# eridgd/WCT-TF

Hardware: AMD Instinct MI355X
Metric: stylized frames/sec @512x512, 5-level relu5->1 pipeline, alpha=0.8 (higher is better)
Workload: dtype f16

## Files before the change

### wct_tf_amd/csrc/conv_wino.hip

```cpp
#include "common.h"

namespace {
typedef unsigned int u32x4 __attribute__((ext_vector_type(4)));
typedef _Float16 h2 __attribute__((ext_vector_type(2)));
constexpr int TW = 16;
constexpr int PITCH = 20;
constexpr int BK = 32;

__device__ __forceinline__ half8 pk_sub(half8 a, half8 b) {
  u32x4 ua = __builtin_bit_cast(u32x4, a), ub = __builtin_bit_cast(u32x4, b), r;
#pragma unroll
  for (int i = 0; i < 4; ++i) {
    unsigned o;
    asm("v_pk_add_f16 %0, %1, %2 neg_lo:[0,1] neg_hi:[0,1]" : "=v"(o) : "v"(ua[i]), "v"(ub[i]));
    r[i] = o;
  }
  return __builtin_bit_cast(half8, r);
}

__device__ __forceinline__ int reflect_idx(int i, int n) {
  if (i < 0) i = -i;
  if (i >= n) i = 2 * n - 2 - i;
  i = i < 0 ? 0 : i;
  return i >= n ? n - 1 : i;
}

template <int TH, int BN, int WM, int WN, bool IL>
__global__ __launch_bounds__(256, TH >= 16 ? 1 : 2)
void conv3x3_wino_kernel(ConvArgs p, int tiles_x, int n_tiles) {
  constexpr int PR = TH / 2;
  constexpr int MT = (PR / 2) / WM;
  constexpr int NT = (BN / 32) / WN;
  constexpr int G = 256 / PR;
  constexpr int SL = (72 + G - 1) / G;
  constexpr int PATCH_BYTES = PR * 4 * PITCH * 64;
  constexpr int DUMP_OFF = 2 * PATCH_BYTES;
  constexpr int PF_TAP = 5;
  static_assert(PR % 2 == 0 && (PR / 2) % WM == 0 && 256 % PR == 0 && WM * WN == 4, "tile shape");

  extern __shared__ __attribute__((aligned(16))) unsigned char smem[];
  const int tid = threadIdx.x, lane = tid & 63, wave = tid >> 6;
  const int wm = wave / WN, wn = wave % WN;
  int bid = blockIdx.x;
  const int ntile = bid % n_tiles;
  bid /= n_tiles;
  const int tx = bid % tiles_x, ty = bid / tiles_x;
  const int b = blockIdx.y;
  const int y0 = ty * TH, x0 = tx * TW, n0 = ntile * BN;

  const int Hin = p.upsample ? p.H / 2 : p.H;
  const int Win = p.upsample ? p.W / 2 : p.W;
  const half_t* xb = p.x + (size_t)b * Hin * Win * p.Cin;
  const __amdgpu_buffer_rsrc_t w_rsrc = __builtin_amdgcn_make_buffer_rsrc((void*)p.w_wino, 0, 0x7FFFFFFF, 0x00020000);
  const __amdgpu_buffer_rsrc_t x_rsrc = __builtin_amdgcn_make_buffer_rsrc((void*)xb, 0, 0x7FFFFFFF, 0x00020000);

  const int lpr = tid / G, ls = tid % G;
  unsigned row_off[4], col_off[SL], dst_off[SL];
  bool slot_ok[SL];
#pragma unroll
  for (int i = 0; i < 4; ++i) {
    int iy = reflect_idx(y0 + 2 * lpr - 1 + i, p.H);
    if (p.upsample) iy >>= 1;
    row_off[i] = (unsigned)(iy * Win) * p.Cin * 2;
  }
#pragma unroll
  for (int j = 0; j < SL; ++j) {
    const int slot = ls + j * G;
    slot_ok[j] = slot < 72;
    const int px = slot_ok[j] ? slot >> 2 : 0, piece = slot & 3;
    int ix = reflect_idx(x0 - 1 + px, p.W);
    if (p.upsample) ix >>= 1;
    col_off[j] = (unsigned)(ix * p.Cin + piece * 8) * 2;
    dst_off[j] = ((lpr * 4 * PITCH + px) * 4 + (piece ^ ((px >> 2) & 3))) * 16;
    if (IL && !slot_ok[j]) dst_off[j] = DUMP_OFF + tid * 16;
  }
  u32x4 raw[SL][4];
  auto load_rows = [&](int chunk) {
#pragma unroll
    for (int j = 0; j < SL; ++j)
#pragma unroll
      for (int i = 0; i < 4; ++i)
        raw[j][i] = __builtin_amdgcn_raw_buffer_load_b128(x_rsrc, row_off[i] + col_off[j], chunk * BK * 2, 0);
  };
  auto park_rows = [&](int buf) {
#pragma unroll
    for (int j = 0; j < SL; ++j) {
      const half8 d0 = __builtin_bit_cast(half8, raw[j][0]), d1 = __builtin_bit_cast(half8, raw[j][1]);
      const half8 d2 = __builtin_bit_cast(half8, raw[j][2]), d3 = __builtin_bit_cast(half8, raw[j][3]);
      const half8 t0 = pk_sub(d0, d2), t1 = d1 + d2, t2 = pk_sub(d2, d1), t3 = pk_sub(d1, d3);
      if (slot_ok[j]) {
        unsigned char* d = smem + buf * PATCH_BYTES + dst_off[j];
        *reinterpret_cast<half8*>(d) = t0;
        *reinterpret_cast<half8*>(d + PITCH * 64) = t1;
        *reinterpret_cast<half8*>(d + 2 * PITCH * 64) = t2;
        *reinterpret_cast<half8*>(d + 3 * PITCH * 64) = t3;
      }
    }
  };

  const int frag_px = lane & 15, frag_pr = (lane & 31) >> 4, kgrp = lane >> 5;
  int rd_base[3][2];
#pragma unroll
  for (int kx = 0; kx < 3; ++kx)
#pragma unroll
    for (int ks = 0; ks < 2; ++ks) {
      const int px = frag_px + kx;
      rd_base[kx][ks] = (((wm * MT * 2 + frag_pr) * 4) * PITCH + px) * 64 + (((ks * 2 + kgrp) ^ ((px >> 2) & 3)) * 16);
    }
  const int c16 = p.Cin >> 4;
  unsigned wfrag[NT];
#pragma unroll
  for (int nt = 0; nt < NT; ++nt) wfrag[nt] = (((n0 >> 5) + wn * NT + nt) * 12 * c16 * 512 + lane * 8) * 2;

  f32x16 acc[4][NT][MT];
#pragma unroll
  for (int nt = 0; nt < NT; ++nt) {
    f32x4 bv[4];
#pragma unroll
    for (int rq = 0; rq < 4; ++rq) bv[rq] = *reinterpret_cast<const f32x4*>(p.bias + n0 + (wn * NT + nt) * 32 + 8 * rq + 4 * kgrp);
#pragma unroll
    for (int f = 0; f < 4; ++f)
#pragma unroll
      for (int mt = 0; mt < MT; ++mt)
#pragma unroll
        for (int r = 0; r < 16; ++r) acc[f][nt][mt][r] = f == 1 ? bv[r >> 2][r & 3] : 0.f;
  }

  const int n_chunks = p.Cin / BK;
  half8 wf[3][NT][2];
  half8 bf[IL ? 3 : 2][2][MT];
  auto load_w = [&](half8 (&dst)[NT][2], int tap12, int chunk) {
    const int soff = (tap12 * c16 + chunk * 2) * 1024;
#pragma unroll
    for (int nt = 0; nt < NT; ++nt)
#pragma unroll
      for (int ks = 0; ks < 2; ++ks)
        dst[nt][ks] = __builtin_bit_cast(half8, __builtin_amdgcn_raw_buffer_load_b128(w_rsrc, wfrag[nt] + ks * 1024, soff, 0));
  };
  auto read_b = [&](half8 (&dst)[2][MT], int f, int kx, int buf) {
#pragma unroll
    for (int ks = 0; ks < 2; ++ks)
#pragma unroll
      for (int mt = 0; mt < MT; ++mt)
        dst[ks][mt] = *reinterpret_cast<const half8*>(smem + buf * PATCH_BYTES + rd_base[kx][ks] + (mt * 8 + f) * PITCH * 64);
  };

  if constexpr (IL) {
    constexpr int NM = 2 * MT * NT;
    constexpr int NR = 2 * NT + 2 * MT;
#ifndef WINO_LT0
#define WINO_LT0 1
#define WINO_PT0 6
#endif
    constexpr int LT0 = WINO_LT0, PT0 = WINO_PT0;
    static_assert(LT0 + SL <= PT0 && PT0 + SL <= 10, "staging schedule");
#ifndef WINO_WRING
#define WINO_WRING 4
#endif
#ifndef WINO_ABL
#define WINO_ABL 0
#endif
#ifndef WINO_RAW_AUX
#define WINO_RAW_AUX 0
#endif
    constexpr int ABL = WINO_ABL;
    constexpr int WR = WINO_WRING, WA = WR - 1;
    static_assert(24 % WR == 0, "ring");
    half8 wq[WR][NT][2];
    half8 tq[4];
    load_rows(0);
#pragma unroll
    for (int i = 0; i < WA; ++i) load_w(wq[i], i, 0);
#pragma unroll
    for (int j = 0; j < SL; ++j) {
      const half8 d0 = __builtin_bit_cast(half8, raw[j][0]), d1 = __builtin_bit_cast(half8, raw[j][1]);
      const half8 d2 = __builtin_bit_cast(half8, raw[j][2]), d3 = __builtin_bit_cast(half8, raw[j][3]);
      unsigned char* d = smem + dst_off[j];
      *reinterpret_cast<half8*>(d) = pk_sub(d0, d2);
      *reinterpret_cast<half8*>(d + PITCH * 64) = d1 + d2;
      *reinterpret_cast<half8*>(d + 2 * PITCH * 64) = pk_sub(d2, d1);
      *reinterpret_cast<half8*>(d + 3 * PITCH * 64) = pk_sub(d1, d3);
    }
    asm volatile("s_waitcnt lgkmcnt(0)\n\ts_barrier" ::: "memory");
    read_b(bf[0], 0, 0, 0);
    read_b(bf[1], 0, 1, 0);
#pragma unroll 1
    for (int pair = 0; pair < n_chunks; pair += 2) {
#pragma unroll
      for (int t = 0; t < 24; ++t) {
        const int tt = t % 12, chunk_i = pair + t / 12, buf = t / 12;
        const int f = tt / 3, kx = tt % 3;
        const int chunk_n = chunk_i + 1 < n_chunks ? chunk_i + 1 : chunk_i;
        const int t3 = (tt + WA) % 12, c3 = tt + WA >= 12 ? chunk_n : chunk_i;
        const int t1 = (tt + 2) % 12, buf1 = tt >= 10 ? buf ^ 1 : buf;
        const int soff3 = (t3 * c16 + c3 * 2) * 1024;
#pragma unroll
        for (int j = 0; j < NM; ++j) {
          const int ks = j / (MT * NT), mt = (j / NT) % MT, nt = j % NT;
          if (!(ABL & 4)) acc[f][nt][mt] = __builtin_amdgcn_mfma_f32_32x32x16_f16(wq[t % WR][nt][ks], bf[t % 3][ks][mt], acc[f][nt][mt], 0, 0, 0);
          else asm volatile("" :: "v"(wq[t % WR][nt][ks]), "v"(bf[t % 3][ks][mt]));
#pragma unroll
          for (int k = j * NR / NM; k < (j + 1) * NR / NM; ++k) {
            if (k < 2 * NT) {
              if (!(ABL & 1)) wq[(t + WA) % WR][k / 2][k % 2] =
                  __builtin_bit_cast(half8, __builtin_amdgcn_raw_buffer_load_b128(w_rsrc, wfrag[k / 2] + (k % 2) * 1024, soff3, 0));
            } else {
              const int kk = k - 2 * NT, ks1 = kk / MT, mt1 = kk % MT;
              if (!(ABL & 8)) bf[(t + 2) % 3][ks1][mt1] = *reinterpret_cast<const half8*>(smem + buf1 * PATCH_BYTES + rd_base[t1 % 3][ks1] + (mt1 * 8 + t1 / 3) * PITCH * 64);
            }
          }
          if (tt >= LT0 && tt < LT0 + SL) {
            const int sl = tt - LT0;
            if (j < 4 && !(ABL & 2)) raw[sl][j] = __builtin_amdgcn_raw_buffer_load_b128(x_rsrc, (ABL & 64) ? (lane & 3) * 16 + j * 64 + sl * 256 : row_off[j] + col_off[sl], (ABL & 32) ? 0 : chunk_n * BK * 2, WINO_RAW_AUX);
          }
          if (tt >= PT0 && tt < PT0 + SL && !(ABL & 16)) {
            const int sl = tt - PT0;
            {
#pragma unroll
              for (int it = j * 8 / NM; it < (j + 1) * 8 / NM; ++it) {
                const int fq = it >> 1;
                if ((it & 1) == 0) {
                  const half8 da = __builtin_bit_cast(half8, raw[sl][fq == 0 ? 0 : fq == 1 ? 1 : fq == 2 ? 2 : 1]);
                  const half8 db = __builtin_bit_cast(half8, raw[sl][fq == 0 ? 2 : fq == 1 ? 2 : fq == 2 ? 1 : 3]);
                  tq[fq] = fq == 1 ? da + db : pk_sub(da, db);
                } else {
                  *reinterpret_cast<half8*>(smem + (buf ^ 1) * PATCH_BYTES * (slot_ok[sl] ? 1 : 0) + dst_off[sl] + fq * PITCH * 64) = tq[fq];
                }
              }
            }
          }
          __builtin_amdgcn_sched_barrier(0);
        }
        if (tt == 9) asm volatile("s_waitcnt lgkmcnt(0)\n\ts_barrier" ::: "memory");
      }
    }
  } else {
  load_rows(0);
  load_w(wf[0], 0, 0);
  load_w(wf[1], 1, 0);
  park_rows(0);
  asm volatile("s_waitcnt lgkmcnt(0)\n\ts_barrier" ::: "memory");
  read_b(bf[0], 0, 0, 0);

#pragma unroll 1
  for (int pair = 0; pair < n_chunks; pair += 2) {
#pragma unroll
    for (int t = 0; t < 24; ++t) {
      const int tt = t % 12, chunk_i = pair + t / 12, buf = t / 12;
      const int f = tt / 3, kx = tt % 3;
      const bool more = chunk_i + 1 < n_chunks;
      {
        const int t2 = (tt + 2) % 12;
        const int c2 = tt + 2 >= 12 ? (more ? chunk_i + 1 : chunk_i) : chunk_i;
        load_w(wf[(t + 2) % 3], t2, c2);
      }
      if (tt == PF_TAP && more) load_rows(chunk_i + 1);
      if (tt != 11) read_b(bf[(t + 1) & 1], (tt + 1) / 3, (tt + 1) % 3, buf);
      else if (more) read_b(bf[(t + 1) & 1], 0, 0, buf ^ 1);
      __builtin_amdgcn_sched_barrier(0);
#pragma unroll
      for (int ks = 0; ks < 2; ++ks)
#pragma unroll
        for (int mt = 0; mt < MT; ++mt)
#pragma unroll
          for (int nt = 0; nt < NT; ++nt)
            acc[f][nt][mt] = __builtin_amdgcn_mfma_f32_32x32x16_f16(wf[t % 3][nt][ks], bf[t & 1][ks][mt], acc[f][nt][mt], 0, 0, 0);
      __builtin_amdgcn_sched_barrier(0);
      if (tt == 10 && more) {
        park_rows(buf ^ 1);
        asm volatile("s_waitcnt lgkmcnt(0)\n\ts_barrier" ::: "memory");
      }
    }
  }

  }
  constexpr int OOB = (int)0x80000000u;
  const int Ho = p.pool ? (p.H + 1) / 2 : p.H, Wo = p.pool ? (p.W + 1) / 2 : p.W;
  const unsigned img_elems = (unsigned)Ho * Wo * p.Cout;
  const __amdgpu_buffer_rsrc_t r16 = __builtin_amdgcn_make_buffer_rsrc((void*)(p.y16 + (size_t)b * img_elems), 0, img_elems * 2, 0x00020000);
  const float lo1 = p.relu ? 0.f : -__builtin_inff();
  const h2 lo2 = {(half_t)lo1, (half_t)lo1};
  const h2 zero2 = {(half_t)0.f, (half_t)0.f};
  const int ox = x0 + frag_px;
  const int chan = n0 + wn * NT * 32;
#pragma unroll
  for (int mt = 0; mt < MT; ++mt) {
    const int oy = y0 + ((wm * MT + mt) * 2 + frag_pr) * 2;
    const bool in0 = (oy < p.H) & (ox < p.W), in1 = (oy + 1 < p.H) & (ox < p.W);
    int off[2];
    if (p.pool) {
      off[0] = in0 && (frag_px & 1) == 0 ? (((oy >> 1) * Wo + (ox >> 1)) * p.Cout + chan + 8 * kgrp) * 2 : OOB;
      off[1] = OOB;
    } else {
      off[0] = in0 ? ((oy * p.W + ox) * p.Cout + chan + 8 * kgrp) * 2 : OOB;
      off[1] = in1 ? (((oy + 1) * p.W + ox) * p.Cout + chan + 8 * kgrp) * 2 : OOB;
    }
#pragma unroll
    for (int nt = 0; nt < NT; ++nt) {
      unsigned pk[2][4][2];
#pragma unroll
      for (int rq = 0; rq < 4; ++rq) {
        f32x4 e, o;
#pragma unroll
        for (int j = 0; j < 4; ++j) {
          const int r = rq * 4 + j;
          const float m0 = acc[0][nt][mt][r], m1 = acc[1][nt][mt][r], m2 = acc[2][nt][mt][r], m3 = acc[3][nt][mt][r];
          e[j] = (m0 + m1) + m2;
          o[j] = (m1 - m2) - m3;
        }
        h2 e0 = {(half_t)e[0], (half_t)e[1]}, e1 = {(half_t)e[2], (half_t)e[3]};
        h2 o0 = {(half_t)o[0], (half_t)o[1]}, o1 = {(half_t)o[2], (half_t)o[3]};
        e0 = __builtin_elementwise_max(e0, lo2); e1 = __builtin_elementwise_max(e1, lo2);
        o0 = __builtin_elementwise_max(o0, lo2); o1 = __builtin_elementwise_max(o1, lo2);
        if (p.pool) {
          h2 q[2] = {__builtin_elementwise_max(in0 ? e0 : zero2, in1 ? o0 : zero2), __builtin_elementwise_max(in0 ? e1 : zero2, in1 ? o1 : zero2)};
#pragma unroll
          for (int d = 0; d < 2; ++d) {
            const unsigned tq = __builtin_bit_cast(unsigned, q[d]);
            const h2 nb = __builtin_bit_cast(h2, __builtin_amdgcn_update_dpp(0, (int)tq, 0xB1, 0xF, 0xF, true));
            q[d] = __builtin_elementwise_max(q[d], nb);
          }
          e0 = q[0]; e1 = q[1];
        }
        pk[0][rq][0] = __builtin_bit_cast(unsigned, e0); pk[0][rq][1] = __builtin_bit_cast(unsigned, e1);
        pk[1][rq][0] = __builtin_bit_cast(unsigned, o0); pk[1][rq][1] = __builtin_bit_cast(unsigned, o1);
      }
#pragma unroll
      for (int par = 0; par < 2; ++par) {
#pragma unroll
        for (int m = 0; m < 2; ++m) {
          auto sx = __builtin_amdgcn_permlane32_swap(pk[par][2 * m][0], pk[par][2 * m + 1][0], false, false);
          auto sy = __builtin_amdgcn_permlane32_swap(pk[par][2 * m][1], pk[par][2 * m + 1][1], false, false);
          u32x4 ov = {sx[0], sy[0], sx[1], sy[1]};
          __builtin_amdgcn_raw_buffer_store_b128(ov, r16, off[par] + (nt * 32 + 16 * m) * 2, 0, 0);
        }
      }
    }
  }
}

template <int TH, int BN, int WM, int WN, bool IL = false>
int launch_wino_cfg(const ConvArgs& a, hipStream_t s) {
  const int tiles_x = cdiv(a.W, TW), tiles_y = cdiv(a.H, TH), n_tiles = a.Cout / BN;
  const size_t lds = 2 * (size_t)(TH / 2) * 4 * PITCH * 64 + (IL ? 8192 : 0);
  HIP_TRY(hipFuncSetAttribute(reinterpret_cast<const void*>(&conv3x3_wino_kernel<TH, BN, WM, WN, IL>),
                              hipFuncAttributeMaxDynamicSharedMemorySize, (int)lds));
  hipLaunchKernelGGL((conv3x3_wino_kernel<TH, BN, WM, WN, IL>), dim3(tiles_x * tiles_y * n_tiles, a.B), dim3(256), lds, s, a, tiles_x, n_tiles);
  HIP_TRY(hipGetLastError());
  return WCT_OK;
}
}

bool conv3x3_wino_takes(const ConvArgs& a) {
  return a.w_wino != nullptr && a.y16 != nullptr && a.y32 == nullptr && a.usum == nullptr && a.img1 == nullptr &&
         a.Cin % 64 == 0 && a.Cout % 64 == 0 && (!a.pool || a.relu);
}

int launch_conv3x3_wino(const ConvArgs& a, hipStream_t s) {
  ARG_CHECK(conv3x3_wino_takes(a) && a.H > 1 && a.W > 1 && a.B > 0);
  ARG_CHECK(!a.upsample || (a.H % 2 == 0 && a.W % 2 == 0));
  ARG_CHECK((size_t)a.H * a.W * a.Cin * 2 < ((size_t)1 << 31));
  ARG_CHECK((size_t)a.H * a.W * a.Cout * 2 < ((size_t)1 << 31));
  const long px16 = (long)cdiv(a.W, TW) * cdiv(a.H, 16) * a.B;
  const long px8 = (long)cdiv(a.W, TW) * cdiv(a.H, 8) * a.B;
  if (a.Cout % 128 == 0 && px16 * (a.Cout / 128) >= 256) return launch_wino_cfg<16, 128, 1, 4, true>(a, s);
  if (a.Cout % 128 == 0 && px8 * (a.Cout / 128) >= 256) return launch_wino_cfg<8, 128, 1, 4>(a, s);
  return launch_wino_cfg<8, 64, 2, 2>(a, s);
}
```

Before: 673.3.

## Specialize Winograd conv for nearest-upsampled input to drop duplicate rows

Adds an UP template variant of the F(2,3) Winograd conv kernel for convolutions whose input is 2x nearest-upsampled. Because row pairs are duplicated, the row input transform collapses to two loaded rows and three frequency planes instead of four, which cuts global loads, LDS footprint and the MFMA tap count by a quarter. Weight taps are remapped so the third plane uses the original fourth transformed weight. It is enabled by default and can be turned off with an environment variable, at the cost of a more complex staging schedule and constant tuning for the new path.

```diff
diff --git a/wct_tf_amd/csrc/conv_wino.hip b/wct_tf_amd/csrc/conv_wino.hip
--- a/wct_tf_amd/csrc/conv_wino.hip
+++ b/wct_tf_amd/csrc/conv_wino.hip
@@ -25,17 +25,23 @@
   return i >= n ? n - 1 : i;
 }
 
-template <int TH, int BN, int WM, int WN, bool IL>
+template <int TH, int BN, int WM, int WN, bool IL, bool UP>
 __global__ __launch_bounds__(256, TH >= 16 ? 1 : 2)
 void conv3x3_wino_kernel(ConvArgs p, int tiles_x, int n_tiles) {
+  constexpr int NF = UP ? 3 : 4;
+  constexpr int NTAP = NF * 3;
+  constexpr int NROW = UP ? 2 : 4;
+  constexpr int RPP = UP ? 2 : 4;
+  auto WF = [](int fi) constexpr { return UP && fi == 2 ? 3 : fi; };
   constexpr int PR = TH / 2;
   constexpr int MT = (PR / 2) / WM;
   constexpr int NT = (BN / 32) / WN;
   constexpr int G = 256 / PR;
-  constexpr int SL = (72 + G - 1) / G;
-  constexpr int PATCH_BYTES = PR * 4 * PITCH * 64;
+  constexpr int LR = UP ? PR + 1 : PR;
+  constexpr int SL = UP ? (LR * 72 + 255) / 256 : (72 + G - 1) / G;
+  constexpr int PATCH_BYTES = LR * RPP * PITCH * 64;
   constexpr int DUMP_OFF = 2 * PATCH_BYTES;
-  constexpr int PF_TAP = 5;
+  constexpr int PF_TAP = NTAP - 7;
   static_assert(PR % 2 == 0 && (PR / 2) % WM == 0 && 256 % PR == 0 && WM * WN == 4, "tile shape");
 
   extern __shared__ __attribute__((aligned(16))) unsigned char smem[];
@@ -48,52 +54,84 @@
   const int b = blockIdx.y;
   const int y0 = ty * TH, x0 = tx * TW, n0 = ntile * BN;
 
-  const int Hin = p.upsample ? p.H / 2 : p.H;
-  const int Win = p.upsample ? p.W / 2 : p.W;
+  const bool ups = UP || p.upsample;
+  const int Hin = ups ? p.H / 2 : p.H;
+  const int Win = ups ? p.W / 2 : p.W;
   const half_t* xb = p.x + (size_t)b * Hin * Win * p.Cin;
   const __amdgpu_buffer_rsrc_t w_rsrc = __builtin_amdgcn_make_buffer_rsrc((void*)p.w_wino, 0, 0x7FFFFFFF, 0x00020000);
   const __amdgpu_buffer_rsrc_t x_rsrc = __builtin_amdgcn_make_buffer_rsrc((void*)xb, 0, 0x7FFFFFFF, 0x00020000);
 
   const int lpr = tid / G, ls = tid % G;
-  unsigned row_off[4], col_off[SL], dst_off[SL];
+  unsigned row_off[4], col_off[SL], dst_off[SL], src_up[SL][2];
   bool slot_ok[SL];
-#pragma unroll
-  for (int i = 0; i < 4; ++i) {
-    int iy = reflect_idx(y0 + 2 * lpr - 1 + i, p.H);
-    if (p.upsample) iy >>= 1;
-    row_off[i] = (unsigned)(iy * Win) * p.Cin * 2;
-  }
-#pragma unroll
-  for (int j = 0; j < SL; ++j) {
-    const int slot = ls + j * G;
-    slot_ok[j] = slot < 72;
-    const int px = slot_ok[j] ? slot >> 2 : 0, piece = slot & 3;
-    int ix = reflect_idx(x0 - 1 + px, p.W);
-    if (p.upsample) ix >>= 1;
-    col_off[j] = (unsigned)(ix * p.Cin + piece * 8) * 2;
-    dst_off[j] = ((lpr * 4 * PITCH + px) * 4 + (piece ^ ((px >> 2) & 3))) * 16;
-    if (IL && !slot_ok[j]) dst_off[j] = DUMP_OFF + tid * 16;
-  }
+  if constexpr (!UP) {
+#pragma unroll
+    for (int i = 0; i < 4; ++i) {
+      int iy = reflect_idx(y0 + 2 * lpr - 1 + i, p.H);
+      if (ups) iy >>= 1;
+      row_off[i] = (unsigned)(iy * Win) * p.Cin * 2;
+    }
+#pragma unroll
+    for (int j = 0; j < SL; ++j) {
+      const int slot = ls + j * G;
+      slot_ok[j] = slot < 72;
+      const int px = slot_ok[j] ? slot >> 2 : 0, piece = slot & 3;
+      int ix = reflect_idx(x0 - 1 + px, p.W);
+      if (ups) ix >>= 1;
+      col_off[j] = (unsigned)(ix * p.Cin + piece * 8) * 2;
+      dst_off[j] = ((lpr * 4 * PITCH + px) * 4 + (piece ^ ((px >> 2) & 3))) * 16;
+      if (IL && !slot_ok[j]) dst_off[j] = DUMP_OFF + tid * 16;
+    }
+  } else {
+#pragma unroll
+    for (int j = 0; j < SL; ++j) {
+      const int item = tid + j * 256;
+      slot_ok[j] = item < LR * 72;
+      const int it = slot_ok[j] ? item : 0;
+      const int lr = it / 72, slot = it - lr * 72;
+      const int px = slot >> 2, piece = slot & 3;
+      const int ix = reflect_idx(x0 - 1 + px, p.W) >> 1;
+#pragma unroll
+      for (int i = 0; i < 2; ++i) {
+        const int iy = reflect_idx(y0 + 2 * lr - 1 + i, p.H) >> 1;
+        src_up[j][i] = (unsigned)((iy * Win + ix) * p.Cin + piece * 8) * 2;
+      }
+      dst_off[j] = ((lr * RPP * PITCH + px) * 4 + (piece ^ ((px >> 2) & 3))) * 16;
+      if (IL && !slot_ok[j]) dst_off[j] = DUMP_OFF + tid * 16;
+    }
+  }
+  auto src_off = [&](int j, int i) -> unsigned {
+    if constexpr (UP) return src_up[j][i]; else return row_off[i] + col_off[j];
+  };
   u32x4 raw[SL][4];
   auto load_rows = [&](int chunk) {
 #pragma unroll
     for (int j = 0; j < SL; ++j)
 #pragma unroll
-      for (int i = 0; i < 4; ++i)
-        raw[j][i] = __builtin_amdgcn_raw_buffer_load_b128(x_rsrc, row_off[i] + col_off[j], chunk * BK * 2, 0);
+      for (int i = 0; i < NROW; ++i)
+        raw[j][i] = __builtin_amdgcn_raw_buffer_load_b128(x_rsrc, src_off(j, i), chunk * BK * 2, 0);
   };
   auto park_rows = [&](int buf) {
 #pragma unroll
     for (int j = 0; j < SL; ++j) {
       const half8 d0 = __builtin_bit_cast(half8, raw[j][0]), d1 = __builtin_bit_cast(half8, raw[j][1]);
-      const half8 d2 = __builtin_bit_cast(half8, raw[j][2]), d3 = __builtin_bit_cast(half8, raw[j][3]);
-      const half8 t0 = pk_sub(d0, d2), t1 = d1 + d2, t2 = pk_sub(d2, d1), t3 = pk_sub(d1, d3);
-      if (slot_ok[j]) {
-        unsigned char* d = smem + buf * PATCH_BYTES + dst_off[j];
-        *reinterpret_cast<half8*>(d) = t0;
-        *reinterpret_cast<half8*>(d + PITCH * 64) = t1;
-        *reinterpret_cast<half8*>(d + 2 * PITCH * 64) = t2;
-        *reinterpret_cast<half8*>(d + 3 * PITCH * 64) = t3;
+      if constexpr (UP) {
+        const half8 t0 = pk_sub(d0, d1), t1 = d1 + d1;
+        if (slot_ok[j]) {
+          unsigned char* d = smem + buf * PATCH_BYTES + dst_off[j];
+          *reinterpret_cast<half8*>(d) = t0;
+          *reinterpret_cast<half8*>(d + PITCH * 64) = t1;
+        }
+      } else {
+        const half8 d2 = __builtin_bit_cast(half8, raw[j][2]), d3 = __builtin_bit_cast(half8, raw[j][3]);
+        const half8 t0 = pk_sub(d0, d2), t1 = d1 + d2, t2 = pk_sub(d2, d1), t3 = pk_sub(d1, d3);
+        if (slot_ok[j]) {
+          unsigned char* d = smem + buf * PATCH_BYTES + dst_off[j];
+          *reinterpret_cast<half8*>(d) = t0;
+          *reinterpret_cast<half8*>(d + PITCH * 64) = t1;
+          *reinterpret_cast<half8*>(d + 2 * PITCH * 64) = t2;
+          *reinterpret_cast<half8*>(d + 3 * PITCH * 64) = t3;
+        }
       }
     }
   };
@@ -105,21 +143,21 @@
 #pragma unroll
     for (int ks = 0; ks < 2; ++ks) {
       const int px = frag_px + kx;
-      rd_base[kx][ks] = (((wm * MT * 2 + frag_pr) * 4) * PITCH + px) * 64 + (((ks * 2 + kgrp) ^ ((px >> 2) & 3)) * 16);
+      rd_base[kx][ks] = (((wm * MT * 2 + frag_pr) * RPP) * PITCH + px) * 64 + (((ks * 2 + kgrp) ^ ((px >> 2) & 3)) * 16);
     }
   const int c16 = p.Cin >> 4;
   unsigned wfrag[NT];
 #pragma unroll
   for (int nt = 0; nt < NT; ++nt) wfrag[nt] = (((n0 >> 5) + wn * NT + nt) * 12 * c16 * 512 + lane * 8) * 2;
 
-  f32x16 acc[4][NT][MT];
+  f32x16 acc[NF][NT][MT];
 #pragma unroll
   for (int nt = 0; nt < NT; ++nt) {
     f32x4 bv[4];
 #pragma unroll
     for (int rq = 0; rq < 4; ++rq) bv[rq] = *reinterpret_cast<const f32x4*>(p.bias + n0 + (wn * NT + nt) * 32 + 8 * rq + 4 * kgrp);
 #pragma unroll
-    for (int f = 0; f < 4; ++f)
+    for (int f = 0; f < NF; ++f)
 #pragma unroll
       for (int mt = 0; mt < MT; ++mt)
 #pragma unroll
@@ -142,7 +180,7 @@
     for (int ks = 0; ks < 2; ++ks)
 #pragma unroll
       for (int mt = 0; mt < MT; ++mt)
-        dst[ks][mt] = *reinterpret_cast<const half8*>(smem + buf * PATCH_BYTES + rd_base[kx][ks] + (mt * 8 + f) * PITCH * 64);
+        dst[ks][mt] = *reinterpret_cast<const half8*>(smem + buf * PATCH_BYTES + rd_base[kx][ks] + (mt * 2 * RPP + f) * PITCH * 64);
   };
 
   if constexpr (IL) {
@@ -152,8 +190,8 @@
 #define WINO_LT0 1
 #define WINO_PT0 6
 #endif
-    constexpr int LT0 = WINO_LT0, PT0 = WINO_PT0;
-    static_assert(LT0 + SL <= PT0 && PT0 + SL <= 10, "staging schedule");
+    constexpr int LT0 = UP ? 0 : WINO_LT0, PT0 = UP ? 4 : WINO_PT0;
+    static_assert(LT0 + SL <= PT0 && PT0 + SL <= NTAP - 2, "staging schedule");
 #ifndef WINO_WRING
 #define WINO_WRING 4
 #endif
@@ -164,22 +202,27 @@
 #define WINO_RAW_AUX 0
 #endif
     constexpr int ABL = WINO_ABL;
-    constexpr int WR = WINO_WRING, WA = WR - 1;
-    static_assert(24 % WR == 0, "ring");
+    constexpr int WR = UP ? 6 : WINO_WRING, WA = UP ? 3 : WR - 1;
+    static_assert((2 * NTAP) % WR == 0 && WA < WR, "ring");
     half8 wq[WR][NT][2];
     half8 tq[4];
     load_rows(0);
 #pragma unroll
-    for (int i = 0; i < WA; ++i) load_w(wq[i], i, 0);
+    for (int i = 0; i < WA; ++i) load_w(wq[i], WF(i / 3) * 3 + i % 3, 0);
 #pragma unroll
     for (int j = 0; j < SL; ++j) {
       const half8 d0 = __builtin_bit_cast(half8, raw[j][0]), d1 = __builtin_bit_cast(half8, raw[j][1]);
-      const half8 d2 = __builtin_bit_cast(half8, raw[j][2]), d3 = __builtin_bit_cast(half8, raw[j][3]);
       unsigned char* d = smem + dst_off[j];
-      *reinterpret_cast<half8*>(d) = pk_sub(d0, d2);
-      *reinterpret_cast<half8*>(d + PITCH * 64) = d1 + d2;
-      *reinterpret_cast<half8*>(d + 2 * PITCH * 64) = pk_sub(d2, d1);
-      *reinterpret_cast<half8*>(d + 3 * PITCH * 64) = pk_sub(d1, d3);
+      if constexpr (UP) {
+        *reinterpret_cast<half8*>(d) = pk_sub(d0, d1);
+        *reinterpret_cast<half8*>(d + PITCH * 64) = d1 + d1;
+      } else {
+        const half8 d2 = __builtin_bit_cast(half8, raw[j][2]), d3 = __builtin_bit_cast(half8, raw[j][3]);
+        *reinterpret_cast<half8*>(d) = pk_sub(d0, d2);
+        *reinterpret_cast<half8*>(d + PITCH * 64) = d1 + d2;
+        *reinterpret_cast<half8*>(d + 2 * PITCH * 64) = pk_sub(d2, d1);
+        *reinterpret_cast<half8*>(d + 3 * PITCH * 64) = pk_sub(d1, d3);
+      }
     }
     asm volatile("s_waitcnt lgkmcnt(0)\n\ts_barrier" ::: "memory");
     read_b(bf[0], 0, 0, 0);
@@ -187,17 +230,17 @@
 #pragma unroll 1
     for (int pair = 0; pair < n_chunks; pair += 2) {
 #pragma unroll
-      for (int t = 0; t < 24; ++t) {
-        const int tt = t % 12, chunk_i = pair + t / 12, buf = t / 12;
-        const int f = tt / 3, kx = tt % 3;
+      for (int t = 0; t < 2 * NTAP; ++t) {
+        const int tt = t % NTAP, chunk_i = pair + t / NTAP, buf = t / NTAP;
+        const int fi = tt / 3;
         const int chunk_n = chunk_i + 1 < n_chunks ? chunk_i + 1 : chunk_i;
-        const int t3 = (tt + WA) % 12, c3 = tt + WA >= 12 ? chunk_n : chunk_i;
-        const int t1 = (tt + 2) % 12, buf1 = tt >= 10 ? buf ^ 1 : buf;
-        const int soff3 = (t3 * c16 + c3 * 2) * 1024;
+        const int t3 = (tt + WA) % NTAP, c3 = tt + WA >= NTAP ? chunk_n : chunk_i;
+        const int t1 = (tt + 2) % NTAP, buf1 = tt >= NTAP - 2 ? buf ^ 1 : buf;
+        const int soff3 = ((WF(t3 / 3) * 3 + t3 % 3) * c16 + c3 * 2) * 1024;
 #pragma unroll
         for (int j = 0; j < NM; ++j) {
           const int ks = j / (MT * NT), mt = (j / NT) % MT, nt = j % NT;
-          if (!(ABL & 4)) acc[f][nt][mt] = __builtin_amdgcn_mfma_f32_32x32x16_f16(wq[t % WR][nt][ks], bf[t % 3][ks][mt], acc[f][nt][mt], 0, 0, 0);
+          if (!(ABL & 4)) acc[fi][nt][mt] = __builtin_amdgcn_mfma_f32_32x32x16_f16(wq[t % WR][nt][ks], bf[t % 3][ks][mt], acc[fi][nt][mt], 0, 0, 0);
           else asm volatile("" :: "v"(wq[t % WR][nt][ks]), "v"(bf[t % 3][ks][mt]));
 #pragma unroll
           for (int k = j * NR / NM; k < (j + 1) * NR / NM; ++k) {
@@ -206,22 +249,22 @@
                   __builtin_bit_cast(half8, __builtin_amdgcn_raw_buffer_load_b128(w_rsrc, wfrag[k / 2] + (k % 2) * 1024, soff3, 0));
             } else {
               const int kk = k - 2 * NT, ks1 = kk / MT, mt1 = kk % MT;
-              if (!(ABL & 8)) bf[(t + 2) % 3][ks1][mt1] = *reinterpret_cast<const half8*>(smem + buf1 * PATCH_BYTES + rd_base[t1 % 3][ks1] + (mt1 * 8 + t1 / 3) * PITCH * 64);
+              if (!(ABL & 8)) bf[(t + 2) % 3][ks1][mt1] = *reinterpret_cast<const half8*>(smem + buf1 * PATCH_BYTES + rd_base[t1 % 3][ks1] + (mt1 * 2 * RPP + t1 / 3) * PITCH * 64);
             }
           }
           if (tt >= LT0 && tt < LT0 + SL) {
             const int sl = tt - LT0;
-            if (j < 4 && !(ABL & 2)) raw[sl][j] = __builtin_amdgcn_raw_buffer_load_b128(x_rsrc, (ABL & 64) ? (lane & 3) * 16 + j * 64 + sl * 256 : row_off[j] + col_off[sl], (ABL & 32) ? 0 : chunk_n * BK * 2, WINO_RAW_AUX);
+            if (j < NROW && !(ABL & 2)) raw[sl][j] = __builtin_amdgcn_raw_buffer_load_b128(x_rsrc, (ABL & 64) ? (lane & 3) * 16 + j * 64 + sl * 256 : src_off(sl, j), (ABL & 32) ? 0 : chunk_n * BK * 2, WINO_RAW_AUX);
           }
           if (tt >= PT0 && tt < PT0 + SL && !(ABL & 16)) {
             const int sl = tt - PT0;
             {
 #pragma unroll
-              for (int it = j * 8 / NM; it < (j + 1) * 8 / NM; ++it) {
+              for (int it = j * 2 * RPP / NM; it < (j + 1) * 2 * RPP / NM; ++it) {
                 const int fq = it >> 1;
                 if ((it & 1) == 0) {
                   const half8 da = __builtin_bit_cast(half8, raw[sl][fq == 0 ? 0 : fq == 1 ? 1 : fq == 2 ? 2 : 1]);
-                  const half8 db = __builtin_bit_cast(half8, raw[sl][fq == 0 ? 2 : fq == 1 ? 2 : fq == 2 ? 1 : 3]);
+                  const half8 db = __builtin_bit_cast(half8, raw[sl][UP ? 1 : fq == 0 ? 2 : fq == 1 ? 2 : fq == 2 ? 1 : 3]);
                   tq[fq] = fq == 1 ? da + db : pk_sub(da, db);
                 } else {
                   *reinterpret_cast<half8*>(smem + (buf ^ 1) * PATCH_BYTES * (slot_ok[sl] ? 1 : 0) + dst_off[sl] + fq * PITCH * 64) = tq[fq];
@@ -231,7 +274,7 @@
           }
           __builtin_amdgcn_sched_barrier(0);
         }
-        if (tt == 9) asm volatile("s_waitcnt lgkmcnt(0)\n\ts_barrier" ::: "memory");
+        if (tt == NTAP - 3) asm volatile("s_waitcnt lgkmcnt(0)\n\ts_barrier" ::: "memory");
       }
     }
   } else {
@@ -245,17 +288,17 @@
 #pragma unroll 1
   for (int pair = 0; pair < n_chunks; pair += 2) {
 #pragma unroll
-    for (int t = 0; t < 24; ++t) {
-      const int tt = t % 12, chunk_i = pair + t / 12, buf = t / 12;
-      const int f = tt / 3, kx = tt % 3;
+    for (int t = 0; t < 2 * NTAP; ++t) {
+      const int tt = t % NTAP, chunk_i = pair + t / NTAP, buf = t / NTAP;
+      const int f = tt / 3;
       const bool more = chunk_i + 1 < n_chunks;
       {
-        const int t2 = (tt + 2) % 12;
-        const int c2 = tt + 2 >= 12 ? (more ? chunk_i + 1 : chunk_i) : chunk_i;
-        load_w(wf[(t + 2) % 3], t2, c2);
+        const int t2 = (tt + 2) % NTAP;
+        const int c2 = tt + 2 >= NTAP ? (more ? chunk_i + 1 : chunk_i) : chunk_i;
+        load_w(wf[(t + 2) % 3], WF(t2 / 3) * 3 + t2 % 3, c2);
       }
       if (tt == PF_TAP && more) load_rows(chunk_i + 1);
-      if (tt != 11) read_b(bf[(t + 1) & 1], (tt + 1) / 3, (tt + 1) % 3, buf);
+      if (tt != NTAP - 1) read_b(bf[(t + 1) & 1], (tt + 1) / 3, (tt + 1) % 3, buf);
       else if (more) read_b(bf[(t + 1) & 1], 0, 0, buf ^ 1);
       __builtin_amdgcn_sched_barrier(0);
 #pragma unroll
@@ -266,7 +309,7 @@
           for (int nt = 0; nt < NT; ++nt)
             acc[f][nt][mt] = __builtin_amdgcn_mfma_f32_32x32x16_f16(wf[t % 3][nt][ks], bf[t & 1][ks][mt], acc[f][nt][mt], 0, 0, 0);
       __builtin_amdgcn_sched_barrier(0);
-      if (tt == 10 && more) {
+      if (tt == NTAP - 2 && more) {
         park_rows(buf ^ 1);
         asm volatile("s_waitcnt lgkmcnt(0)\n\ts_barrier" ::: "memory");
       }
@@ -304,9 +347,15 @@
 #pragma unroll
         for (int j = 0; j < 4; ++j) {
           const int r = rq * 4 + j;
-          const float m0 = acc[0][nt][mt][r], m1 = acc[1][nt][mt][r], m2 = acc[2][nt][mt][r], m3 = acc[3][nt][mt][r];
-          e[j] = (m0 + m1) + m2;
-          o[j] = (m1 - m2) - m3;
+          const float m0 = acc[0][nt][mt][r], m1 = acc[1][nt][mt][r], m3 = acc[NF - 1][nt][mt][r];
+          if (UP) {
+            e[j] = m0 + m1;
+            o[j] = m1 - m3;
+          } else {
+            const float m2 = acc[2][nt][mt][r];
+            e[j] = (m0 + m1) + m2;
+            o[j] = (m1 - m2) - m3;
+          }
         }
         h2 e0 = {(half_t)e[0], (half_t)e[1]}, e1 = {(half_t)e[2], (half_t)e[3]};
         h2 o0 = {(half_t)o[0], (half_t)o[1]}, o1 = {(half_t)o[2], (half_t)o[3]};
@@ -339,15 +388,26 @@
   }
 }
 
+template <int TH, int BN, int WM, int WN, bool IL, bool UP>
+int launch_wino_up(const ConvArgs& a, hipStream_t s) {
+  const int tiles_x = cdiv(a.W, TW), tiles_y = cdiv(a.H, TH), n_tiles = a.Cout / BN;
+  const size_t lds = 2 * (size_t)(UP ? TH / 2 + 1 : TH / 2) * (UP ? 2 : 4) * PITCH * 64 + (IL ? 8192 : 0);
+  HIP_TRY(hipFuncSetAttribute(reinterpret_cast<const void*>(&conv3x3_wino_kernel<TH, BN, WM, WN, IL, UP>),
+                              hipFuncAttributeMaxDynamicSharedMemorySize, (int)lds));
+  hipLaunchKernelGGL((conv3x3_wino_kernel<TH, BN, WM, WN, IL, UP>), dim3(tiles_x * tiles_y * n_tiles, a.B), dim3(256), lds, s, a, tiles_x, n_tiles);
+  HIP_TRY(hipGetLastError());
+  return WCT_OK;
+}
+
+bool upsample_dedup() {
+  static const int on = getenv("WCT_UPSAMPLE_DEDUP") ? atoi(getenv("WCT_UPSAMPLE_DEDUP")) : 1;
+  return on != 0;
+}
+
 template <int TH, int BN, int WM, int WN, bool IL = false>
 int launch_wino_cfg(const ConvArgs& a, hipStream_t s) {
-  const int tiles_x = cdiv(a.W, TW), tiles_y = cdiv(a.H, TH), n_tiles = a.Cout / BN;
-  const size_t lds = 2 * (size_t)(TH / 2) * 4 * PITCH * 64 + (IL ? 8192 : 0);
-  HIP_TRY(hipFuncSetAttribute(reinterpret_cast<const void*>(&conv3x3_wino_kernel<TH, BN, WM, WN, IL>),
-                              hipFuncAttributeMaxDynamicSharedMemorySize, (int)lds));
-  hipLaunchKernelGGL((conv3x3_wino_kernel<TH, BN, WM, WN, IL>), dim3(tiles_x * tiles_y * n_tiles, a.B), dim3(256), lds, s, a, tiles_x, n_tiles);
-  HIP_TRY(hipGetLastError());
-  return WCT_OK;
+  if (a.upsample && upsample_dedup()) return launch_wino_up<TH, BN, WM, WN, IL, true>(a, s);
+  return launch_wino_up<TH, BN, WM, WN, IL, false>(a, s);
 }
 }
 
```

Result: no change. 676.2 (median of 6 runs) (+0.4%).
